# douban/tfmesos

Measured on AMD Instinct MI355X. Metric: global steps/sec, mnist_replica 1-ps/N-worker at 1/2/4/8 MI355X, higher is better.
Workload: dtype bf16; 1 GPU; model=mnist_replica_mlp_784x100x10, global_batch=100, parallelism=ps1+w1(colocated), optimizer=sgd, sync=True, transport=none(colocated-1proc)

## Files before the change

### tfmesos_amd/ops/csrc/gemm.hip

```cpp
#include <cstdlib>

#include "common.h"
#include "gemm.h"
#include "mlp_head.h"

namespace {

constexpr int BM = 64, BN = 64, BK = 32;
constexpr int SWZ_ELEMS = BM * BK;

DEVINL __bf16* sptr(__bf16* S, int r, int c) {
  return S + r * BK + ((((c >> 3) ^ ((r >> 2) & 3)) << 3) | (c & 7));
}
DEVINL const __bf16* sptr(const __bf16* S, int r, int c) {
  return S + r * BK + ((((c >> 3) ^ ((r >> 2) & 3)) << 3) | (c & 7));
}

typedef __attribute__((ext_vector_type(2))) __bf16 bf16x2;

DEVINL void stage_xk(const __bf16* __restrict__ P, __bf16* S,
                     int x0, int k0, int X, int K, int ld, int t, int vec) {
  const int x = t >> 2;
  const int kk0 = (t & 3) * 8;
  const int gx = x0 + x;
// ... 558 lines not shown
    for (int z2 = 0; z2 < nslice; ++z2)
      v += __builtin_bit_cast(
          float, *(const bf16x2*)&f1_smem[z2 * (G::WAVE_BYTES / 2) + e * 2]);
    if (bias != nullptr)
      v += e == t ? bv
                  : (bias_bf16 ? (float)((const __bf16*)bias)[col]
                               : ((const float*)bias)[col]);
    if (relu) v = v > 0.f ? v : 0.f;
    const long idx = (long)row * ldc + col;
    if (out_f32) ((float*)Cout)[idx] = v;
    else ((__bf16*)Cout)[idx] = (__bf16)v;
  }
}

typedef __attribute__((ext_vector_type(16))) float f32x16;

struct SmallSgd {
  float* pmw;
  bf16_t* psw;
  float* pmb;
  bf16_t* psb;
  const bf16_t* g2w;
  float* pm2w;
  bf16_t* ps2w;
  const bf16_t* g2b;
  float* pm2b;
  bf16_t* ps2b;
  float lr;
  int n2w, n2b;
};

DEVINL bf16x8 trs_frag(const __bf16* S, int ko, int lane) {
  const int kq = ko + ((lane & 15) >> 2);
  const int c = 16 * ((lane >> 4) & 1) + 4 * (lane & 3);
  bf16x4 f0 = tr_read(sptr(S, kq, c));
  bf16x4 f1 = tr_read(sptr(S, kq + 4, c));
  return __builtin_shufflevector(f0, f1, 0, 1, 2, 3, 4, 5, 6, 7);
}

DEVINL void small_cs_reduce(const float* csp, float* csw, int lane) {
  float c2[16];
#pragma unroll
  for (int j = 0; j < 16; ++j) c2[j] = csp[j];
#pragma unroll
  for (int off = 1; off < 32; off <<= 1)
#pragma unroll
    for (int j = 0; j < 16; ++j) c2[j] += __shfl_xor(c2[j], off, 64);
  if ((lane & 31) == 0) {
#pragma unroll
    for (int j = 0; j < 16; ++j) csw[(lane >> 5) * 16 + j] = c2[j];
  }
}

struct SmallSgdPre {
  float w[4];
  float b;
};

DEVINL void wait_vm0() { __builtin_amdgcn_s_waitcnt(0x0F70); }
DEVINL void wait_lgkm0() { __builtin_amdgcn_s_waitcnt(0xC07F); }

DEVINL int small_sgd_row(int m0, int w, int u, int lane) {
  const int v = w * 4 + u;
  return m0 + ((v >> 2) << 3) + ((lane >> 5) << 2) + (v & 3);
}

DEVINL void small_sgd_fetch(const SmallSgd& sg, SmallSgdPre& pre, bool cs,
                            int m0, int n0, int M, int N, int ldc, int w,
                            int lane) {
  const int n = n0 + (lane & 31);
#pragma unroll
  for (int u = 0; u < 4; ++u) {
    const int m = small_sgd_row(m0, w, u, lane);
    const long idx = (n < N && m < M) ? (long)m * ldc + n : 0;
    pre.w[u] = sg.pmw[idx];
  }
  pre.b = 0.f;
  if (cs && blockIdx.x == 0 && sg.pmb != nullptr) {
    const int nn = n0 + (lane & 31);
    pre.b = sg.pmb[nn < N ? nn : 0];
  }
}

DEVINL void small_sgd_fetch_buf(const SmallSgd& sg, SmallSgdPre& pre, int m0,
                                int n0, int M, int N, int w, int lane) {
  const brsrc_t wr = buf_rsrc(sg.pmw, M * N * 4);
  const int n = n0 + (lane & 31);
  const int nb = n < N ? n * 4 : BUF_OOB;
#pragma unroll
  for (int u = 0; u < 4; ++u)
    pre.w[u] = buf_f32(wr, nb + small_sgd_row(m0, w, u, lane) * N * 4);
  pre.b = 0.f;
  if (blockIdx.x == 0 && sg.pmb != nullptr)
    pre.b = buf_f32(buf_rsrc(sg.pmb, N * 4), n * 4);
}

DEVINL void small_sgd_commit(const SmallSgd& sg, const SmallSgdPre& pre,
                             const float (*red)[64 * 16],
                             const float (*csred)[32], bool cs, int m0,
                             int n0, int M, int N, int ldc, int w, int lane) {
  const int n = n0 + (lane & 31);
  if (n < N) {
#pragma unroll
    for (int u = 0; u < 4; ++u) {
      const int v = w * 4 + u;
      const int m = small_sgd_row(m0, w, u, lane);
      if (m >= M) continue;
      const float x = red[0][lane * 16 + v] + red[1][lane * 16 + v] +
                      red[2][lane * 16 + v] + red[3][lane * 16 + v];
      const long idx = (long)m * ldc + n;
      const float pv = pre.w[u] - sg.lr * x;
      sg.pmw[idx] = pv;
      sg.psw[idx] = f2bf(pv);
    }
  }
  if (cs && w == 0 && blockIdx.x == 0 && lane < 32) {
    const int nn = n0 + lane;
    if (nn < N && sg.pmb != nullptr) {
      const float sv = csred[0][lane] + csred[1][lane] + csred[2][lane] +
                       csred[3][lane];
      const float pv = pre.b - sg.lr * sv;
      sg.pmb[nn] = pv;
      sg.psb[nn] = f2bf(pv);
    }
  }
}

DEVINL void small_store(const float (*red)[64 * 16],
                        const float (*csred)[32], bool cs,
                        const void* bias, bool bias_bf16, void* Cout,
                        bool out_f32, int relu, void* colsum_out,
                        bool cs_f32, int m0, int n0, int M, int N, int ldc,
                        int lane) {
  f32x16 tot;
#pragma unroll
  for (int v = 0; v < 16; ++v)
    tot[v] = red[0][lane * 16 + v] + red[1][lane * 16 + v] +
             red[2][lane * 16 + v] + red[3][lane * 16 + v];
  const int n = n0 + (lane & 31);
  if (n < N) {
    float bvv = 0.f;
    if (bias != nullptr)
      bvv = bias_bf16 ? (float)((const __bf16*)bias)[n]
                      : ((const float*)bias)[n];
#pragma unroll
    for (int v = 0; v < 16; ++v) {
      const int m = m0 + ((v >> 2) << 3) + ((lane >> 5) << 2) + (v & 3);
      if (m >= M) continue;
      float x = tot[v] + bvv;
      if (relu) x = x > 0.f ? x : 0.f;
      if (out_f32) ((float*)Cout)[(long)m * ldc + n] = x;
      else ((__bf16*)Cout)[(long)m * ldc + n] = (__bf16)x;
    }
  }
  if (cs && blockIdx.x == 0 && lane < 32) {
    const int nn = n0 + lane;
    if (nn < N) {
      const float sv = csred[0][lane] + csred[1][lane] + csred[2][lane] +
                       csred[3][lane];
      if (cs_f32) ((float*)colsum_out)[nn] = sv;
      else ((__bf16*)colsum_out)[nn] = (__bf16)sv;
    }
  }
}

template <bool TA, bool CS>
__global__ __launch_bounds__(256)
void gemm_small_kernel(const __bf16* __restrict__ A,
                       const __bf16* __restrict__ B,
                       const void* __restrict__ bias, bool bias_bf16,
                       void* __restrict__ Cout, bool out_f32, int relu,
                       void* __restrict__ colsum_out, bool cs_f32,
                       int M, int N, int K, int lda, int ldb, int ldc,
                       int veca, int vecb, SmallSgd sg) {
  __shared__ __align__(16) __bf16 As[4][32 * BK];
  __shared__ __align__(16) __bf16 Bs[4][32 * BK];
  __shared__ float red[4][64 * 16];
  __shared__ float csred[4][32];
  const int t = threadIdx.x;
  const int lane = t & 63;
  const int w = t >> 6;
  const int m0 = blockIdx.x * 32;
  const int n0 = blockIdx.y * 32;
  const int kq = (((K + 3) / 4) + BK - 1) / BK * BK;
  const int ks = w * kq;
  const int ke = min(ks + kq, K);
  __bf16* Aw = As[w];
  __bf16* Bw = Bs[w];
  const int kk = lane & 31;
  const int half = lane >> 5;
  const bool av = veca == 8;
  const bool bv = vecb == 8;
  f32x4 acc[4] = {};
  float csp[16] = {};
  bf16x8 ra0, ra1, rb0, rb1;
  SmallSgdPre pre = {};
  if (sg.pmw != nullptr)
    small_sgd_fetch(sg, pre, CS, m0, n0, M, N, ldc, w, lane);

  auto load_a = [&](int k0) {
    ra0 = bf16x8{};
    ra1 = bf16x8{};
    if (TA) {
      const int gk = k0 + kk;
      const int gm = m0 + half * 16;
      if (gk < ke) {
        const __bf16* src = A + (long)gk * lda + gm;
        if (av && gm + 16 <= M && ((m0 & 7) == 0)) {
          ra0 = *(const bf16x8*)src;
          ra1 = *(const bf16x8*)(src + 8);
        } else {
#pragma unroll
          for (int j = 0; j < 8; ++j) {
            if (gm + j < M) ra0[j] = src[j];
            if (gm + 8 + j < M) ra1[j] = src[8 + j];
          }
        }
      }
    } else {
      const int gm = m0 + kk;
      const int gk0 = k0 + half * 16;
      if (gm < M) {
        const __bf16* src = A + (long)gm * lda + gk0;
        if (av && gk0 + 16 <= ke) {
          ra0 = *(const bf16x8*)src;
          ra1 = *(const bf16x8*)(src + 8);
        } else {
#pragma unroll
          for (int j = 0; j < 8; ++j) {
            if (gk0 + j < ke) ra0[j] = src[j];
            if (gk0 + 8 + j < ke) ra1[j] = src[8 + j];
          }
        }
      }
    }
    rb0 = bf16x8{};
    rb1 = bf16x8{};
    {
      const int gk = k0 + kk;
      const int gn = n0 + half * 16;
      if (gk < ke) {
        const __bf16* src = B + (long)gk * ldb + gn;
        if (bv && gn + 16 <= N && ((n0 & 7) == 0)) {
          rb0 = *(const bf16x8*)src;
          rb1 = *(const bf16x8*)(src + 8);
        } else {
// ... 48 lines not shown
    bf16x4 gv[4] = {};
    if (nv > 0) {
#pragma unroll
      for (int u = 0; u < 4; ++u) {
        const int i = lane + u * 64;
        gv[u] = ((const bf16x4*)sg.g2w)[i < nv ? i : 0];
        mv[u] = ((const f32x4*)sg.pm2w)[i < nv ? i : 0];
      }
    }
    const int it = (nv << 2) + lane;
    const int itc = it < sg.n2w ? it : 0;
    const int ibc = lane < sg.n2b ? lane : 0;
    const float mt = sg.pm2w[itc];
    const bf16_t gt = sg.g2w[itc];
    const float mb = sg.pm2b[ibc];
    const bf16_t gb = sg.g2b[ibc];
    wait_vm0();
#pragma unroll
    for (int u = 0; u < 4; ++u) {
      const int i = lane + u * 64;
      if (i < nv) {
        f32x4 pv;
        bf16x4 sv;
#pragma unroll
        for (int j = 0; j < 4; ++j) {
          pv[j] = mv[u][j] - sg.lr * (float)gv[u][j];
          sv[j] = (__bf16)pv[j];
        }
        ((f32x4*)sg.pm2w)[i] = pv;
        ((bf16x4*)sg.ps2w)[i] = sv;
      }
    }
    for (int i = 256 + lane; i < nv; i += 64) {
      f32x4 pv;
      bf16x4 sv;
      const bf16x4 g = ((const bf16x4*)sg.g2w)[i];
      const f32x4 m = ((const f32x4*)sg.pm2w)[i];
#pragma unroll
      for (int j = 0; j < 4; ++j) {
        pv[j] = m[j] - sg.lr * (float)g[j];
        sv[j] = (__bf16)pv[j];
      }
      ((f32x4*)sg.pm2w)[i] = pv;
      ((bf16x4*)sg.ps2w)[i] = sv;
    }
    if (it < sg.n2w) {
      const float pv = mt - sg.lr * bf2f(gt);
      sg.pm2w[it] = pv;
      sg.ps2w[it] = f2bf(pv);
    }
    if (lane < sg.n2b) {
      const float pv = mb - sg.lr * bf2f(gb);
      sg.pm2b[lane] = pv;
      sg.ps2b[lane] = f2bf(pv);
    }
    for (int i = lane + 64; i < sg.n2b; i += 64) {
      const float pv = sg.pm2b[i] - sg.lr * bf2f(sg.g2b[i]);
      sg.pm2b[i] = pv;
      sg.ps2b[i] = f2bf(pv);
    }
  }
  if (sg.pmw != nullptr) {
    small_sgd_commit(sg, pre, red, csred, CS, m0, n0, M, N, ldc, w, lane);
    return;
  }
  if (w != 0) return;
  small_store(red, csred, CS, bias, bias_bf16, Cout, out_f32, relu,
              colsum_out, cs_f32, m0, n0, M, N, ldc, lane);
}

struct HeadTail {
  const __bf16* h;
  const __bf16* w2;
  const bf16_t* b2;
  const long* labels;
  float* loss;
  void* dw2;
  void* db2;
  unsigned* ticket;
  float scale;
  int C;
};

template <bool APPLY, bool GF32, bool SNAP>
__global__ __launch_bounds__(256)
void mlp_head_tail_kernel(const __bf16* __restrict__ X, HeadTail ht,
                          void* __restrict__ Cout,
                          void* __restrict__ colsum_out,
                          int M, int N, int K, SmallSgd sg) {
  __shared__ __align__(16) __bf16 hs[HB * HP];
  __shared__ __align__(16) __bf16 wtp[4][CP * HP];
  __shared__ __align__(16) __bf16 wpd[4][32 * CP];
  __shared__ __align__(16) __bf16 dls[HB * CP];
  __shared__ float ls[HB * LSP];
  __shared__ float lsum[HB];
  __shared__ __align__(16) __bf16 As[4][32 * BK];
  __shared__ __align__(16) __bf16 Bs[4][32 * BK];
  __shared__ float red[4][64 * 16];
  __shared__ float csred[4][32];
  __shared__ float db2p[CP * 16];
  __shared__ unsigned tick;
  const int t = threadIdx.x;
  const int lane = t & 63;
  const int w = t >> 6;
  const int m0 = blockIdx.x * 32;
  const int n0 = blockIdx.y * 32;
  const int C = ht.C;
  const int ks = w * 32;
  const int ke = min(ks + 32, K);
  __bf16* Aw = As[w];
  __bf16* Bw = Bs[w];
  __bf16* wtw = wtp[w];
  __bf16* wpw = wpd[w];
  const int kk = lane & 31;
  const int half = lane >> 5;

  const int gk = ks + kk;
  const int gm = m0 + half * 16;
  const bool xvec = (M & 7) == 0;
  bf16x8 ra0 = {}, ra1 = {};
  unsigned xs[16];
  {
    const brsrc_t xr = buf_rsrc(X, K * M * 2);
    const int xrow = gk * M + gm;
    if (xvec) {
      ra0 = __builtin_bit_cast(bf16x8, __builtin_amdgcn_raw_buffer_load_b128(
          xr, gm < M ? xrow * 2 : BUF_OOB, 0, 0));
      ra1 = __builtin_bit_cast(bf16x8, __builtin_amdgcn_raw_buffer_load_b128(
          xr, gm + 8 < M ? (xrow + 8) * 2 : BUF_OOB, 0, 0));
    } else {
#pragma unroll
      for (int j = 0; j < 16; ++j)
        xs[j] = __builtin_amdgcn_raw_buffer_load_b16(
            xr, gm + j < M ? (xrow + j) * 2 : BUF_OOB, 0, 0);
    }
  }
  const int hc4 = kk * 4;
  bf16x4 hv[16];
  {
    const brsrc_t hr = buf_rsrc(ht.h, K * N * 2);
    const int hb = (hc4 < N ? hc4 * 2 : BUF_OOB) + (ks + half) * N * 2;
#pragma unroll
    for (int i = 0; i < 16; ++i)
      hv[i] = __builtin_bit_cast(bf16x4, __builtin_amdgcn_raw_buffer_load_b64(
          hr, hb + 2 * i * N * 2, 0, 0));
  }
  __bf16 wv[2][CP];
  bf16x8 wkm[4], wrow;
  if (SNAP) {
#pragma unroll
    for (int j = 0; j < 4; ++j) {
      const int q = lane + j * 64;
      wkm[j] = *(const bf16x8*)&ht.w2[kSnapKmajOff + (q >> 4) * HP +
                                      (q & 15) * 8];
    }
    wrow = *(const bf16x8*)&ht.w2[kSnapRowOff + n0 * CP + lane * 8];
  } else {
#pragma unroll
    for (int q = 0; q < 2; ++q) {
      const int hr = lane + q * 64;
#pragma unroll
      for (int c = 0; c < CP; ++c)
        wv[q][c] = ht.w2[(hr < N && c < C) ? hr * C + c : 0];
    }
  }
  const unsigned braw =
      __builtin_amdgcn_raw_buffer_load_b16(buf_rsrc(ht.b2, C * 2), kk * 2, 0, 0);
  const int label = (int)__builtin_amdgcn_raw_buffer_load_b32(
      buf_rsrc(ht.labels, K * 8), (ks + kk) * 8, 0, 0);
  SmallSgdPre pre = {};
  float pm2[16] = {};
  float pm2bv = 0.f;
  const bool snap_head =
      APPLY && SNAP && blockIdx.x == gridDim.x - 1 && blockIdx.y == 0;
  if (APPLY) {
    small_sgd_fetch_buf(sg, pre, m0, n0, M, N, w, lane);
    if (snap_head) {
      const brsrc_t w2r = buf_rsrc(sg.pm2w, N * C * 4);
      const int cb = kk < C ? kk * 4 : BUF_OOB;
#pragma unroll
      for (int v = 0; v < 16; ++v)
        pm2[v] = buf_f32(w2r, cb + (ks + head_frag_row(v, lane)) * C * 4);
      pm2bv = buf_f32(buf_rsrc(sg.pm2b, C * 4), t * 4);
    }
  }

  if (!SNAP) {
#pragma unroll
    for (int q = 0; q < 2; ++q)
#pragma unroll
      for (int c = 0; c < CP; ++c)
        if (!(lane + q * 64 < N && c < C)) wv[q][c] = (__bf16)0.f;
  }
  const float bc = __builtin_bit_cast(float, braw << 16);
  if (!xvec) {
    u32x4 d0, d1;
#pragma unroll
    for (int j = 0; j < 4; ++j) {
      d0[j] = xs[2 * j] | (xs[2 * j + 1] << 16);
      d1[j] = xs[8 + 2 * j] | (xs[9 + 2 * j] << 16);
    }
    ra0 = __builtin_bit_cast(bf16x8, d0);
    ra1 = __builtin_bit_cast(bf16x8, d1);
  }

  if (!SNAP) {
    const bf16x8 z8 = {};
    for (int i = lane * 8; i < CP * HP; i += 64 * 8) *(bf16x8*)&wtw[i] = z8;
    *(bf16x8*)&wpw[lane * 8] = z8;
  }
#pragma unroll
  for (int i = 0; i < 16; ++i)
    *(bf16x4*)&hs[(ks + 2 * i + half) * HP + hc4] = hv[i];
  if (SNAP) {
#pragma unroll
    for (int j = 0; j < 4; ++j) {
      const int q = lane + j * 64;
      *(bf16x8*)&wtw[(q >> 4) * HP + (q & 15) * 8] = wkm[j];
    }
    *(bf16x8*)&wpw[lane * 8] = wrow;
  } else {
#pragma unroll
    for (int q = 0; q < 2; ++q) {
      const int hr = lane + q * 64;
#pragma unroll
      for (int c = 0; c < CP; ++c) wtw[c * HP + hr] = wv[q][c];
      if (hr >= n0 && hr < n0 + 32 && hr < N) {
        bf16x8 lo, hi;
#pragma unroll
        for (int c = 0; c < 8; ++c) {
          lo[c] = wv[q][c];
          hi[c] = wv[q][8 + c];
        }
        *(bf16x8*)&wpw[(hr - n0) * CP] = lo;
        *(bf16x8*)&wpw[(hr - n0) * CP + 8] = hi;
      }
    }
  }

  {
    const f32x16v acc = head_logits_tile(
        &hs[(ks + kk) * HP], kk < CP ? &wtw[kk * HP] : nullptr, lane);
    head_store_logits(ls, acc, ks, bc, lane);
  }
  if (lane < 32) {
    const int row = ks + lane;
    const bf16x8 z8 = {};
    *(bf16x8*)&dls[row * CP] = z8;
    *(bf16x8*)&dls[row * CP + 8] = z8;
    float neglogp = 0.f;
    if (row < K)
      neglogp = head_softmax_row(
          &ls[row * LSP], C, label, ht.scale,
          [&](int c, float d) { dls[row * CP + c] = (__bf16)d; });
    lsum[row] = neglogp;
  }
  {
    const int colh = n0 + kk;
    __bf16 hm[16];
#pragma unroll
    for (int v = 0; v < 16; ++v)
      hm[v] = hs[(ks + head_frag_row(v, lane)) * HP + colh];
    const f32x16v acc =
        head_dh_tile(&dls[(ks + kk) * CP], &wpw[kk * CP], lane);
    wait_lgkm0();
#pragma unroll
    for (int v = 0; v < 16; ++v) {
      const int rl = head_frag_row(v, lane);
      const float hval = (float)hm[v];
      const float m =
          (ks + rl < K && colh < N && hval > 0.f) ? acc[v] : 0.f;
      const bf16_t r = f2bf(m);
      *sptr(Bw, rl, kk) = *(const __bf16*)&r;
    }
  }
  *(bf16x8*)sptr(Aw, kk, half * 16) = ra0;
  *(bf16x8*)sptr(Aw, kk, half * 16 + 8) = ra1;
  if (blockIdx.x == 0) {
    const bf16x8 rb0 = *(const bf16x8*)sptr(Bw, kk, half * 16);
    const bf16x8 rb1 = *(const bf16x8*)sptr(Bw, kk, half * 16 + 8);
    float csp[16] = {};
#pragma unroll
    for (int j = 0; j < 8; ++j) {
      csp[j] += (float)rb0[j];
      csp[8 + j] += (float)rb1[j];
    }
    small_cs_reduce(csp, csred[w], lane);
  }
  f32x4 acc[4] = {};
  if (ks < ke) {
#pragma unroll
    for (int kh = 0; kh < 2; ++kh) {
      const int ko = kh * 16 + ((lane >> 5) << 3);
      bf16x8 a = trs_frag(Aw, ko, lane);
      bf16x8 b = trs_frag(Bw, ko, lane);
      *(f32x16*)acc = __builtin_amdgcn_mfma_f32_32x32x16_bf16(
          a, b, *(f32x16*)acc, 0, 0, 0);
    }
  }
#pragma unroll
  for (int v = 0; v < 16; ++v) red[w][lane * 16 + v] = ((float*)acc)[v];
  __syncthreads();
  wait_vm0();

  bool head_block;
  constexpr bool ticketed = APPLY && !SNAP;
  if (APPLY) {
    if (ticketed && t == 0)
      tick = __hip_atomic_fetch_add(ht.ticket, 1u, __ATOMIC_ACQ_REL,
                                    __HIP_MEMORY_SCOPE_AGENT);
    small_sgd_commit(sg, pre, red, csred, true, m0, n0, M, N, N, w, lane);
    if (ticketed) {
      __syncthreads();
      head_block = tick == gridDim.x * gridDim.y - 1;
      if (head_block) {
#pragma unroll
        for (int v = 0; v < 16; ++v) {
          const int hrow = ks + head_frag_row(v, lane);
          pm2[v] = sg.pm2w[(kk < C && hrow < N) ? hrow * C + kk : 0];
        }
        pm2bv = sg.pm2b[t < C ? t : 0];
        wait_vm0();
      }
    } else {
      head_block = snap_head;
    }
  } else {
    if (gridDim.x * gridDim.y >= 32) {
      if (w == 0)
        small_store(red, csred, true, nullptr, false, Cout, GF32, 0,
                    colsum_out, GF32, m0, n0, M, N, N, lane);
    } else {
      const int wr = w >> 1, wc = w & 1;
      const int kfrag = (lane >> 4) * 8;
      const int kr = kfrag + ((lane & 15) >> 2);
      const int cq = 4 * (lane & 3);
      f32x4 c4 = {};
      for (int q = 0; q * 32 < K; ++q) {
        bf16x4 a0 = tr_read(sptr(As[q], kr, wr * 16 + cq));
        bf16x4 a1 = tr_read(sptr(As[q], kr + 4, wr * 16 + cq));
        bf16x4 b0 = tr_read(sptr(Bs[q], kr, wc * 16 + cq));
        bf16x4 b1 = tr_read(sptr(Bs[q], kr + 4, wc * 16 + cq));
        c4 = __builtin_amdgcn_mfma_f32_16x16x32_bf16(
            __builtin_shufflevector(a0, a1, 0, 1, 2, 3, 4, 5, 6, 7),
            __builtin_shufflevector(b0, b1, 0, 1, 2, 3, 4, 5, 6, 7), c4,
            0, 0, 0);
      }
      const int col = n0 + wc * 16 + (lane & 15);
      if (col < N) {
#pragma unroll
        for (int r = 0; r < 4; ++r) {
          const int row = m0 + wr * 16 + (lane >> 4) * 4 + r;
          if (row >= M) continue;
          float v = c4[r];
          v += 0.f;
          if (GF32) ((float*)Cout)[(long)row * N + col] = v;
          else ((__bf16*)Cout)[(long)row * N + col] = (__bf16)v;
        }
      }
      if (blockIdx.x == 0 && t < 32 && n0 + t < N) {
        float cs = 0.f;
        for (int q = 0; q * 32 < K; ++q)
#pragma unroll
          for (int k2 = 0; k2 < 32; ++k2) cs += (float)*sptr(Bs[q], k2, t);
        if (GF32) ((float*)colsum_out)[n0 + t] = cs;
        else ((__bf16*)colsum_out)[n0 + t] = (__bf16)cs;
      }
    }
    head_block = blockIdx.x == 0 && blockIdx.y == 0;
  }
  if (!head_block) return;

  {
    f32x16v acc2 = {};
    const int kr = (lane & 15) >> 2;
    const int ca = ks + 16 * ((lane >> 4) & 1) + 4 * (lane & 3);
    const int cb = 4 * (lane & 3);
    const bool bzero = ((lane >> 4) & 1) != 0;
#pragma unroll
    for (int kh = 0; kh < HB / 16; ++kh) {
      const int kq = kh * 16 + ((lane >> 5) << 3) + kr;
      bf16x4 a0 = tr_read(&hs[kq * HP + ca]);
      bf16x4 a1 = tr_read(&hs[(kq + 4) * HP + ca]);
      bf16x4 b0 = tr_read(&dls[kq * CP + cb]);
      bf16x4 b1 = tr_read(&dls[(kq + 4) * CP + cb]);
      bf16x8 a = __builtin_shufflevector(a0, a1, 0, 1, 2, 3, 4, 5, 6, 7);
      bf16x8 bv = __builtin_shufflevector(b0, b1, 0, 1, 2, 3, 4, 5, 6, 7);
      if (bzero) bv = bf16x8{};
      acc2 = __builtin_amdgcn_mfma_f32_32x32x16_bf16(a, bv, acc2, 0, 0, 0);
    }
    if (kk < C) {
#pragma unroll
      for (int v = 0; v < 16; ++v) {
        const int hrow = ks + head_frag_row(v, lane);
        if (hrow < N) {
          const int idx = hrow * C + kk;
          if (APPLY) {
            const float pv = pm2[v] - sg.lr * bf2f(f2bf(acc2[v]));
            sg.pm2w[idx] = pv;
            sg.ps2w[idx] = f2bf(pv);
          } else if (GF32) {
            ((float*)ht.dw2)[idx] = acc2[v];
          } else {
            ((bf16_t*)ht.dw2)[idx] = f2bf(acc2[v]);
          }
        }
      }
    }
  }
  if (t < C * 16) {
    const int c = t >> 4, part = t & 15;
    float s = 0.f;
    for (int b2 = part; b2 < K; b2 += 16) s += (float)dls[b2 * CP + c];
    db2p[t] = s;
  }
  __syncthreads();
  if (t < C) {
    float s = 0.f;
#pragma unroll
    for (int p2 = 0; p2 < 16; ++p2) s += db2p[t * 16 + p2];
    if (APPLY) {
      const float pv = pm2bv - sg.lr * bf2f(f2bf(s));
      sg.pm2b[t] = pv;
      sg.ps2b[t] = f2bf(pv);
    } else if (GF32) {
      ((float*)ht.db2)[t] = s;
    } else {
      ((bf16_t*)ht.db2)[t] = f2bf(s);
    }
  }
  if (w == 0) {
    float v = (lsum[lane] + 0.f) + (lsum[lane + 64] + 0.f);
#pragma unroll
    for (int s = 32; s > 0; s >>= 1) v += __shfl_down(v, s, 64);
    if (lane == 0) *ht.loss = v / K;
  }
  if (ticketed && t == 0)
    __hip_atomic_store(ht.ticket, 0u, __ATOMIC_RELAXED,
                       __HIP_MEMORY_SCOPE_AGENT);
}

__global__ __launch_bounds__(256)
void splitk_reduce_sgd_kernel(const float* __restrict__ ws, int nslice,
                              float* __restrict__ p,
                              __bf16* __restrict__ shadow, long mn,
                              float lr, float gscale, float nd) {
  const long i0 = ((long)blockIdx.x * blockDim.x + threadIdx.x) * 4;
  if (i0 >= mn) return;
  const bool vec4 = stripes_vec4(ws, mn);
  f32x4 v = {};
  for (int z = 0; z < nslice; ++z) {
    const float* sp = ws + (long)z * mn + i0;
    if (vec4) {
      const f32x4 sv = *(const f32x4*)sp;
#pragma unroll
      for (int j = 0; j < 4; ++j) v[j] += sv[j];
    } else {
#pragma unroll
      for (int j = 0; j < 4; ++j)
        if (i0 + j < mn) v[j] += sp[j];
    }
  }
#pragma unroll
  for (int j = 0; j < 4; ++j) {
    const long i = i0 + j;
    if (i >= mn) break;
    float pv = p[i];
    float g = gscale * v[j];
    if (nd != 0.f) g += nd * fminf(pv, 0.f);
    pv -= lr * g;
    p[i] = pv;
    if (shadow != nullptr) shadow[i] = (__bf16)pv;
  }
}

}

bool gemm_last_arriver(int M, int N, bool colsum, int act) {
  static int la_on = -1;
  if (la_on < 0) {
    const char* e = getenv("TFA_GEMM_LA");
    la_on = e ? atoi(e) : 0;
  }
  return la_on && !colsum && act <= 1 &&
         (long)ceil_div(N, BN) * ceil_div(M, BM) <= 64;
}

bool gemm_reduce_small(long mn) { return mn <= (1 << 16); }

void launch_gemm(const bf16_t* A, const bf16_t* B, const void* bias,
                 bool bias_bf16, void* C, bool out_f32, const bf16_t* aux,
                 void* colsum_out, float* ws, int* cnt, int kc, int nslice,
                 int M, int N, int K, int lda, int ldb, int ldc, bool ta,
                 bool tb, int act, int veca, int vecb, hipStream_t stream,
                 const SnapArgs* snap, bool* snap_taken) {
  SnapJob sj = {};
  if (snap_taken) *snap_taken = false;
  const bool sk = nslice > 1;
  dim3 grid(ceil_div(N, BN), ceil_div(M, BM), sk ? nslice : 1);
  dim3 block(256);
  const bool has_bias = bias != nullptr;
  const bool cs = colsum_out != nullptr;
  const int rflags = (act == 1 ? 1 : 0) | (out_f32 ? 2 : 0) |
                     (has_bias ? 4 : 0);
  if (!gemm_last_arriver(M, N, cs, act)) cnt = nullptr;
#define LAUNCH(TAv, TBv, ACTv, BIASv, OUTv, SKv, CSv)                       \
  hipLaunchKernelGGL((gemm_kernel<TAv, TBv, ACTv, BIASv, OUTv, SKv, CSv>),  \
                     grid, block, 0, stream, (const __bf16*)A,              \
                     (const __bf16*)B, bias, bias_bf16, C,                  \
                     (const __bf16*)aux, colsum_out, ws, cnt, M, N, K, lda, \
                     ldb, ldc, kc, veca, vecb, rflags)
  if (act == 2) {
    LAUNCH(false, true, 2, false, false, false, false);
    return;
  }
  if (act == 3) {
    LAUNCH(false, false, 3, false, false, false, false);
    return;
  }
  if (cs && !sk) {
    if (out_f32) LAUNCH(true, false, 0, false, true, false, true);
    else         LAUNCH(true, false, 0, false, false, false, true);
// ... 68 lines not shown
       else DISP_OUT(TAv, TBv, ACTv, false); } while (0)
#define DISP_ACT(TAv, TBv)                                                  \
  do { if (act == 1) DISP_BIAS(TAv, TBv, 1); else DISP_BIAS(TAv, TBv, 0); } while (0)
  if (ta) { if (tb) DISP_ACT(true, true); else DISP_ACT(true, false); }
  else    { if (tb) DISP_ACT(false, true); else DISP_ACT(false, false); }
#undef DISP_ACT
#undef DISP_BIAS
#undef DISP_OUT
#undef LAUNCH
}

void launch_gemm_fwd1(const bf16_t* A, const bf16_t* B, const void* bias,
                      bool bias_bf16, void* C, bool out_f32, int relu,
                      int kc, int nslice, int M, int N, int K, int lda,
                      int ldb, int ldc, int veca, int vecb, int variant,
                      const SnapArgs* snap, bool* snap_taken,
                      hipStream_t stream) {
  SnapJob sj = {};
  if (snap != nullptr) {
    sj.s0 = (const __bf16*)snap->s0; sj.s1 = (const __bf16*)snap->s1;
    sj.dst = (__bf16*)snap->dst;
    sj.n0 = snap->n0; sj.n1 = snap->n1; sj.off1 = snap->off1;
    sj.rows = snap->rows; sj.cols = snap->cols;
  }
  if (snap_taken) *snap_taken = snap != nullptr;
  if (variant < 0) variant = kFwd1Tile;
  const bool va = veca == 8 && K % 8 == 0;
  const bool vb = vecb >= 2 && N % 2 == 0 && N >= 8 && !(variant & 4);
  dim3 block(64 * nslice);
#define F1V(TMv, TNv, VAv, VBv)                                             \
  hipLaunchKernelGGL((gemm_fwd1_kernel<TMv, TNv, VAv, VBv>),                \
                     dim3(ceil_div(N, TNv), ceil_div(M, TMv)), block,       \
                     (nslice * (Fwd1Geo<TMv, TNv>::WAVE_BYTES)), stream,    \
                     (const __bf16*)A, (const __bf16*)B, bias, bias_bf16,   \
                     C, out_f32, relu, M, N, K, lda, ldb, ldc, kc, sj)
#define F1(TMv, TNv)                                                        \
  do { if (va) { if (vb) F1V(TMv, TNv, true, true);                         \
                 else F1V(TMv, TNv, true, false); }                         \
       else    { if (vb) F1V(TMv, TNv, false, true);                        \
                 else F1V(TMv, TNv, false, false); } } while (0)
  switch (variant & 3) {
    case 0: F1(16, 16); break;
    case 1: F1(16, 32); break;
    case 2: F1(32, 16); break;
    default: F1(32, 32); break;
  }
#undef F1
#undef F1V
}


void launch_gemm_small(const bf16_t* A, const bf16_t* B, const void* bias,
                       bool bias_bf16, void* C, bool out_f32, int relu,
                       void* colsum_out, bool cs_f32, int M, int N, int K,
                       int lda, int ldb, int ldc, bool ta, int veca,
                       int vecb, const SmallSgdArgs* sga,
                       hipStream_t stream) {
  dim3 grid(ceil_div(M, 32), ceil_div(N, 32)), block(256);
  SmallSgd sg = {};
  if (sga) {
    sg.pmw = sga->pmw; sg.psw = (bf16_t*)sga->psw;
    sg.pmb = sga->pmb; sg.psb = (bf16_t*)sga->psb;
    sg.g2w = (const bf16_t*)sga->g2w;
    sg.pm2w = sga->pm2w; sg.ps2w = (bf16_t*)sga->ps2w;
    sg.g2b = (const bf16_t*)sga->g2b;
    sg.pm2b = sga->pm2b; sg.ps2b = (bf16_t*)sga->ps2b;
    sg.lr = sga->lr; sg.n2w = sga->n2w; sg.n2b = sga->n2b;
  }
  const bool cs = colsum_out != nullptr || sg.pmb != nullptr;
#define GS(TAv, CSv)                                                        \
  hipLaunchKernelGGL((gemm_small_kernel<TAv, CSv>), grid, block, 0,         \
                     stream, (const __bf16*)A, (const __bf16*)B, bias,      \
                     bias_bf16, C, out_f32, relu, colsum_out, cs_f32, M, N, \
                     K, lda, ldb, ldc, veca, vecb, sg)
  if (ta) { if (cs) GS(true, true); else GS(true, false); }
  else    { if (cs) GS(false, true); else GS(false, false); }
#undef GS
}

void launch_mlp_head_tail(const bf16_t* x, const HeadTailArgs* hta,
                          void* dw1, void* db1, bool grads_f32, int M,
                          int H, int B, const SmallSgdArgs* sga,
                          hipStream_t stream) {
  dim3 grid(ceil_div(M, 32), ceil_div(H, 32)), block(256);
  HeadTail ht;
  ht.h = (const __bf16*)hta->h;
  ht.w2 = (const __bf16*)hta->w2;
  ht.b2 = (const bf16_t*)hta->b2;
  ht.labels = hta->labels;
  ht.loss = hta->loss;
  ht.dw2 = hta->dw2;
  ht.db2 = hta->db2;
  ht.ticket = hta->ticket;
  ht.scale = hta->scale;
  ht.C = hta->C;
  SmallSgd sg = {};
  if (sga) {
    sg.pmw = sga->pmw; sg.psw = (bf16_t*)sga->psw;
    sg.pmb = sga->pmb; sg.psb = (bf16_t*)sga->psb;
    sg.pm2w = sga->pm2w; sg.ps2w = (bf16_t*)sga->ps2w;
    sg.pm2b = sga->pm2b; sg.ps2b = (bf16_t*)sga->ps2b;
    sg.lr = sga->lr; sg.n2w = sga->n2w; sg.n2b = sga->n2b;
    if (ht.ticket == nullptr)
      hipLaunchKernelGGL((mlp_head_tail_kernel<true, false, true>), grid,
                         block, 0, stream, (const __bf16*)x, ht, nullptr,
                         nullptr, M, H, B, sg);
    else
      hipLaunchKernelGGL((mlp_head_tail_kernel<true, false, false>), grid,
                         block, 0, stream, (const __bf16*)x, ht, nullptr,
                         nullptr, M, H, B, sg);
  } else if (grads_f32) {
    hipLaunchKernelGGL((mlp_head_tail_kernel<false, true, false>), grid,
                       block, 0, stream, (const __bf16*)x, ht, dw1, db1, M, H,
                       B, sg);
  } else {
    hipLaunchKernelGGL((mlp_head_tail_kernel<false, false, false>), grid,
                       block, 0, stream, (const __bf16*)x, ht, dw1, db1, M, H,
                       B, sg);
  }
}


void launch_gemm_stripes_any(const bf16_t* A, const bf16_t* B, float* ws,
                             int kc, int nslice, int M, int N, int K,
                             int lda, int ldb, int ldc, bool ta, bool tb,
                             int veca, int vecb, hipStream_t stream) {
  const long Mtiles = ((long)M + BM - 1) / BM;
  dim3 grid((unsigned)ceil_div(N, BN), (unsigned)Mtiles, nslice);
  dim3 block(256);
#define SLAUNCH(TAv, TBv)                                                   \
  hipLaunchKernelGGL((gemm_kernel<TAv, TBv, 0, false, false, true, false>), \
                     grid, block, 0, stream, (const __bf16*)A,              \
                     (const __bf16*)B, nullptr, false, nullptr, nullptr,    \
                     nullptr, ws, nullptr, M, N, K, lda, ldb, ldc, kc, veca,\
                     vecb, 0)
  if (ta) { if (tb) SLAUNCH(true, true); else SLAUNCH(true, false); }
  else    { if (tb) SLAUNCH(false, true); else SLAUNCH(false, false); }
#undef SLAUNCH
}

void launch_splitk_reduce_sgd(const float* ws, int nslice, float* p,
                              bf16_t* shadow, long mn, float lr,
                              float gscale, float nd, hipStream_t stream) {
  dim3 rgrid((unsigned)(((mn + 3) / 4 + 255) / 256)), rblock(256);
  hipLaunchKernelGGL(splitk_reduce_sgd_kernel, rgrid, rblock, 0, stream,
                     ws, nslice, p, (__bf16*)shadow, mn, lr, gscale, nd);
}

void launch_gemm_stripes(const bf16_t* A, const bf16_t* B, float* ws,
                         int kc, int nslice, int M, int N, int K, int lda,
                         int ldb, int ldc, int veca, int vecb,
                         hipStream_t stream) {
  dim3 grid(ceil_div(N, BN), ceil_div(M, BM), nslice);
  dim3 block(256);
  hipLaunchKernelGGL((gemm_kernel<false, false, 0, false, false, true,
                                  false>),
                     grid, block, 0, stream, (const __bf16*)A,
                     (const __bf16*)B, nullptr, false, nullptr, nullptr,
                     nullptr, ws, nullptr, M, N, K, lda, ldb, ldc, kc,
                     veca, vecb, 0);
}
```

### tfmesos_amd/ops/csrc/mlp_head.h

```cpp
#pragma once

#include "common.h"

typedef __attribute__((ext_vector_type(16))) float f32x16v;

constexpr int HB = 128;
constexpr int HP = 136;
constexpr int CP = 16;
constexpr int LSP = CP + 1;

DEVINL int head_frag_row(int v, int lane) {
  return ((v >> 2) << 3) + ((lane >> 5) << 2) + (v & 3);
}

DEVINL f32x16v head_logits_tile(const __bf16* arow, const __bf16* brow,
                                int lane) {
  f32x16v acc = {};
#pragma unroll
  for (int kh = 0; kh < HB / 16; ++kh) {
    const int k0 = kh * 16 + ((lane >> 5) << 3);
    bf16x8 a = *(const bf16x8*)&arow[k0];
    bf16x8 bv = {};
    if (brow != nullptr) bv = *(const bf16x8*)&brow[k0];
    acc = __builtin_amdgcn_mfma_f32_32x32x16_bf16(a, bv, acc, 0, 0, 0);
  }
  return acc;
}

DEVINL void head_store_logits(float* ls, const f32x16v& acc, int row0,
                              float bc, int lane) {
  const int col = lane & 31;
  if (col < CP) {
#pragma unroll
    for (int v = 0; v < 16; ++v)
      ls[(row0 + head_frag_row(v, lane)) * LSP + col] = acc[v] + bc;
  }
}

template <class F>
DEVINL float head_softmax_row(const float* lr, int C, int label,
                              float scale, F emit) {
  float l[CP];
#pragma unroll
  for (int c = 0; c < CP; ++c) l[c] = lr[c];
  float mx = -3.4e38f;
#pragma unroll
  for (int c = 0; c < CP; ++c)
    if (c < C) mx = fmaxf(mx, l[c]);
  float sum = 0.f;
  float e[CP];
#pragma unroll
  for (int c = 0; c < CP; ++c) {
    e[c] = 0.f;
    if (c < C) {
      e[c] = __expf(l[c] - mx);
      sum += e[c];
    }
  }
  const float inv = 1.f / sum;
  float pl = 1.f;
  bool hit = false;
#pragma unroll
  for (int c = 0; c < CP; ++c) {
    if (c < C) {
      const float p = e[c] * inv;
      const float d = (p - (c == label ? 1.f : 0.f)) * scale;
      emit(c, d);
      if (c == label) {
        pl = p;
        hit = true;
      }
    }
  }
  return hit ? -__logf(fmaxf(pl, 1e-30f)) : 0.f;
}

DEVINL f32x16v head_dh_tile(const __bf16* drow, const __bf16* wrow,
                            int lane) {
  bf16x8 a = *(const bf16x8*)&drow[(lane >> 5) << 3];
  bf16x8 bv = *(const bf16x8*)&wrow[(lane >> 5) << 3];
  f32x16v acc = {};
  return __builtin_amdgcn_mfma_f32_32x32x16_bf16(a, bv, acc, 0, 0, 0);
}
```

Measured before the change: 56670 steps/s.

## Split fused MLP head-tail kernel into tile, db1 and classifier block roles

Restructures the fused backward head/tail kernel. For the non-ticketed (snapshot) path, it adds two extra grid columns whose blocks take dedicated roles: dW1 tiles, the db1 column-sum/SGD update, and the classifier dW2/db2 work split across two blocks. This keeps the serial head work off the last tile block. It also makes the softmax and logits paths branchless by padding classes with a negative-infinity bias and vectorized bf16 stores, and simplifies the dH masking writes. The cost is extra blocks that redundantly recompute the logits/softmax, plus more shared-memory padding.

New measurement: 65360 steps/s (median of 6 runs). +15.3%, better.

```diff
diff --git a/tfmesos_amd/ops/csrc/gemm.hip b/tfmesos_amd/ops/csrc/gemm.hip
--- a/tfmesos_amd/ops/csrc/gemm.hip
+++ b/tfmesos_amd/ops/csrc/gemm.hip
@@ -664,17 +664,34 @@
   }
 }
 
-DEVINL void small_sgd_fetch_buf(const SmallSgd& sg, SmallSgdPre& pre, int m0,
-                                int n0, int M, int N, int w, int lane) {
+DEVINL void small_sgd_fetch_buf_w(const SmallSgd& sg, SmallSgdPre& pre,
+                                  int m0, int n0, int M, int N, int w,
+                                  int lane) {
   const brsrc_t wr = buf_rsrc(sg.pmw, M * N * 4);
   const int n = n0 + (lane & 31);
   const int nb = n < N ? n * 4 : BUF_OOB;
 #pragma unroll
   for (int u = 0; u < 4; ++u)
     pre.w[u] = buf_f32(wr, nb + small_sgd_row(m0, w, u, lane) * N * 4);
-  pre.b = 0.f;
-  if (blockIdx.x == 0 && sg.pmb != nullptr)
-    pre.b = buf_f32(buf_rsrc(sg.pmb, N * 4), n * 4);
+}
+
+DEVINL void small_sgd_fetch_buf_b(const SmallSgd& sg, SmallSgdPre& pre,
+                                  int n0, int N, int lane) {
+  if (sg.pmb != nullptr)
+    pre.b = buf_f32(buf_rsrc(sg.pmb, N * 4), (n0 + (lane & 31)) * 4);
+}
+
+DEVINL void small_sgd_commit_b(const SmallSgd& sg, const SmallSgdPre& pre,
+                               const float (*csred)[32], int n0, int N,
+                               int lane) {
+  const int nn = n0 + lane;
+  if (nn < N && sg.pmb != nullptr) {
+    const float sv = csred[0][lane] + csred[1][lane] + csred[2][lane] +
+                     csred[3][lane];
+    const float pv = pre.b - sg.lr * sv;
+    sg.pmb[nn] = pv;
+    sg.psb[nn] = f2bf(pv);
+  }
 }
 
 DEVINL void small_sgd_commit(const SmallSgd& sg, const SmallSgdPre& pre,
@@ -696,15 +713,18 @@
       sg.psw[idx] = f2bf(pv);
     }
   }
-  if (cs && w == 0 && blockIdx.x == 0 && lane < 32) {
-    const int nn = n0 + lane;
-    if (nn < N && sg.pmb != nullptr) {
-      const float sv = csred[0][lane] + csred[1][lane] + csred[2][lane] +
-                       csred[3][lane];
-      const float pv = pre.b - sg.lr * sv;
-      sg.pmb[nn] = pv;
-      sg.psb[nn] = f2bf(pv);
-    }
+  if (cs && w == 0 && blockIdx.x == 0 && lane < 32)
+    small_sgd_commit_b(sg, pre, csred, n0, N, lane);
+}
+
+DEVINL void small_store_cs(const float (*csred)[32], void* colsum_out,
+                           bool cs_f32, int n0, int N, int lane) {
+  const int nn = n0 + lane;
+  if (nn < N) {
+    const float sv = csred[0][lane] + csred[1][lane] + csred[2][lane] +
+                     csred[3][lane];
+    if (cs_f32) ((float*)colsum_out)[nn] = sv;
+    else ((__bf16*)colsum_out)[nn] = (__bf16)sv;
   }
 }
 
@@ -735,15 +755,8 @@
       else ((__bf16*)Cout)[(long)m * ldc + n] = (__bf16)x;
     }
   }
-  if (cs && blockIdx.x == 0 && lane < 32) {
-    const int nn = n0 + lane;
-    if (nn < N) {
-      const float sv = csred[0][lane] + csred[1][lane] + csred[2][lane] +
-                       csred[3][lane];
-      if (cs_f32) ((float*)colsum_out)[nn] = sv;
-      else ((__bf16*)colsum_out)[nn] = (__bf16)sv;
-    }
-  }
+  if (cs && blockIdx.x == 0 && lane < 32)
+    small_store_cs(csred, colsum_out, cs_f32, n0, N, lane);
 }
 
 template <bool TA, bool CS>
@@ -958,24 +971,44 @@
   int C;
 };
 
-template <bool APPLY, bool GF32, bool SNAP>
-__global__ __launch_bounds__(256)
-void mlp_head_tail_kernel(const __bf16* __restrict__ X, HeadTail ht,
-                          void* __restrict__ Cout,
-                          void* __restrict__ colsum_out,
-                          int M, int N, int K, SmallSgd sg) {
-  __shared__ __align__(16) __bf16 hs[HB * HP];
-  __shared__ __align__(16) __bf16 wtp[4][CP * HP];
-  __shared__ __align__(16) __bf16 wpd[4][32 * CP];
-  __shared__ __align__(16) __bf16 dls[HB * CP];
-  __shared__ float ls[HB * LSP];
-  __shared__ float lsum[HB];
-  __shared__ __align__(16) __bf16 As[4][32 * BK];
-  __shared__ __align__(16) __bf16 Bs[4][32 * BK];
-  __shared__ float red[4][64 * 16];
-  __shared__ float csred[4][32];
-  __shared__ float db2p[CP * 16];
-  __shared__ unsigned tick;
+enum { HT_ALL = 0, HT_TILE = 1, HT_DB1 = 2, HT_CLS = 3 };
+
+struct HeadTailSmem {
+  alignas(16) __bf16 hs[HB * HP];
+  alignas(16) __bf16 wtp[4][(CP + 1) * HP];
+  alignas(16) __bf16 wpd[4][32 * CP];
+  alignas(16) __bf16 dls[HB * CP];
+  float ls[HB * LSP];
+  float lsum[HB];
+  alignas(16) __bf16 As[4][32 * BK];
+  alignas(16) __bf16 Bs[4][32 * BK];
+  float red[4][64 * 16];
+  float csred[4][32];
+  float db2p[CP * 16];
+  unsigned tick;
+};
+
+template <bool APPLY, bool GF32, bool SNAP, int ROLE>
+DEVINL void head_tail_body(HeadTailSmem& sm, const __bf16* __restrict__ X,
+                           const HeadTail& ht, void* __restrict__ Cout,
+                           void* __restrict__ colsum_out, int M, int N,
+                           int K, const SmallSgd& sg, int tiles) {
+  static_assert(ROLE != HT_ALL || (APPLY && !SNAP), "HT_ALL: ticket only");
+  static_assert(ROLE == HT_ALL || !APPLY || SNAP, "roles need no ticket");
+  constexpr bool TILE = ROLE == HT_ALL || ROLE == HT_TILE;
+  constexpr bool DH = ROLE != HT_CLS;
+  auto& hs = sm.hs;
+  auto& wtp = sm.wtp;
+  auto& wpd = sm.wpd;
+  auto& dls = sm.dls;
+  auto& ls = sm.ls;
+  auto& lsum = sm.lsum;
+  auto& As = sm.As;
+  auto& Bs = sm.Bs;
+  auto& red = sm.red;
+  auto& csred = sm.csred;
+  auto& db2p = sm.db2p;
+  auto& tick = sm.tick;
   const int t = threadIdx.x;
   const int lane = t & 63;
   const int w = t >> 6;
@@ -996,7 +1029,7 @@
   const bool xvec = (M & 7) == 0;
   bf16x8 ra0 = {}, ra1 = {};
   unsigned xs[16];
-  {
+  if (TILE) {
     const brsrc_t xr = buf_rsrc(X, K * M * 2);
     const int xrow = gk * M + gm;
     if (xvec) {
@@ -1030,7 +1063,7 @@
       wkm[j] = *(const bf16x8*)&ht.w2[kSnapKmajOff + (q >> 4) * HP +
                                       (q & 15) * 8];
     }
-    wrow = *(const bf16x8*)&ht.w2[kSnapRowOff + n0 * CP + lane * 8];
+    if (DH) wrow = *(const bf16x8*)&ht.w2[kSnapRowOff + n0 * CP + lane * 8];
   } else {
 #pragma unroll
     for (int q = 0; q < 2; ++q) {
@@ -1047,11 +1080,11 @@
   SmallSgdPre pre = {};
   float pm2[16] = {};
   float pm2bv = 0.f;
-  const bool snap_head =
-      APPLY && SNAP && blockIdx.x == gridDim.x - 1 && blockIdx.y == 0;
   if (APPLY) {
-    small_sgd_fetch_buf(sg, pre, m0, n0, M, N, w, lane);
-    if (snap_head) {
+    if (TILE) small_sgd_fetch_buf_w(sg, pre, m0, n0, M, N, w, lane);
+    if (ROLE == HT_DB1 || (ROLE == HT_ALL && blockIdx.x == 0))
+      small_sgd_fetch_buf_b(sg, pre, n0, N, lane);
+    if (ROLE == HT_CLS) {
       const brsrc_t w2r = buf_rsrc(sg.pm2w, N * C * 4);
       const int cb = kk < C ? kk * 4 : BUF_OOB;
 #pragma unroll
@@ -1068,8 +1101,9 @@
       for (int c = 0; c < CP; ++c)
         if (!(lane + q * 64 < N && c < C)) wv[q][c] = (__bf16)0.f;
   }
-  const float bc = __builtin_bit_cast(float, braw << 16);
-  if (!xvec) {
+  const float bc =
+      kk < C ? __builtin_bit_cast(float, braw << 16) : head_pad_bias();
+  if (TILE && !xvec) {
     u32x4 d0, d1;
 #pragma unroll
     for (int j = 0; j < 4; ++j) {
@@ -1083,25 +1117,26 @@
   if (!SNAP) {
     const bf16x8 z8 = {};
     for (int i = lane * 8; i < CP * HP; i += 64 * 8) *(bf16x8*)&wtw[i] = z8;
-    *(bf16x8*)&wpw[lane * 8] = z8;
+    if (DH) *(bf16x8*)&wpw[lane * 8] = z8;
   }
 #pragma unroll
   for (int i = 0; i < 16; ++i)
     *(bf16x4*)&hs[(ks + 2 * i + half) * HP + hc4] = hv[i];
+  if (lane < HB / 8) *(bf16x8*)&wtw[CP * HP + lane * 8] = bf16x8{};
   if (SNAP) {
 #pragma unroll
     for (int j = 0; j < 4; ++j) {
       const int q = lane + j * 64;
       *(bf16x8*)&wtw[(q >> 4) * HP + (q & 15) * 8] = wkm[j];
     }
-    *(bf16x8*)&wpw[lane * 8] = wrow;
+    if (DH) *(bf16x8*)&wpw[lane * 8] = wrow;
   } else {
 #pragma unroll
     for (int q = 0; q < 2; ++q) {
       const int hr = lane + q * 64;
 #pragma unroll
       for (int c = 0; c < CP; ++c) wtw[c * HP + hr] = wv[q][c];
-      if (hr >= n0 && hr < n0 + 32 && hr < N) {
+      if (DH && hr >= n0 && hr < n0 + 32 && hr < N) {
         bf16x8 lo, hi;
 #pragma unroll
         for (int c = 0; c < 8; ++c) {
@@ -1115,23 +1150,24 @@
   }
 
   {
-    const f32x16v acc = head_logits_tile(
-        &hs[(ks + kk) * HP], kk < CP ? &wtw[kk * HP] : nullptr, lane);
+    const f32x16v acc = head_logits_tile_all(
+        &hs[(ks + kk) * HP], &wtw[min(kk, CP) * HP], lane);
     head_store_logits(ls, acc, ks, bc, lane);
   }
   if (lane < 32) {
     const int row = ks + lane;
-    const bf16x8 z8 = {};
-    *(bf16x8*)&dls[row * CP] = z8;
-    *(bf16x8*)&dls[row * CP + 8] = z8;
     float neglogp = 0.f;
-    if (row < K)
-      neglogp = head_softmax_row(
-          &ls[row * LSP], C, label, ht.scale,
-          [&](int c, float d) { dls[row * CP + c] = (__bf16)d; });
+    if (row < K) {
+      neglogp = head_softmax_row_all(&ls[row * LSP], &dls[row * CP], C, label,
+                                     ht.scale);
+    } else {
+      const bf16x8 z8 = {};
+      *(bf16x8*)&dls[row * CP] = z8;
+      *(bf16x8*)&dls[row * CP + 8] = z8;
+    }
     lsum[row] = neglogp;
   }
-  {
+  if (DH) {
     const int colh = n0 + kk;
     __bf16 hm[16];
 #pragma unroll
@@ -1140,19 +1176,22 @@
     const f32x16v acc =
         head_dh_tile(&dls[(ks + kk) * CP], &wpw[kk * CP], lane);
     wait_lgkm0();
+    const int sw = (kk >> 3) ^ half;
+    __bf16* const bq[2] = {Bw + half * 4 * BK + (sw << 3) + (kk & 7),
+                           Bw + half * 4 * BK + ((sw ^ 2) << 3) + (kk & 7)};
 #pragma unroll
     for (int v = 0; v < 16; ++v) {
-      const int rl = head_frag_row(v, lane);
-      const float hval = (float)hm[v];
-      const float m =
-          (ks + rl < K && colh < N && hval > 0.f) ? acc[v] : 0.f;
+      const float m = (float)hm[v] > 0.f ? acc[v] : 0.f;
       const bf16_t r = f2bf(m);
-      *sptr(Bw, rl, kk) = *(const __bf16*)&r;
-    }
-  }
-  *(bf16x8*)sptr(Aw, kk, half * 16) = ra0;
-  *(bf16x8*)sptr(Aw, kk, half * 16 + 8) = ra1;
-  if (blockIdx.x == 0) {
+      bq[(v >> 2) & 1][((v >> 2) * 8 + (v & 3)) * BK] = *(const __bf16*)&r;
+    }
+  }
+  if (TILE) {
+    *(bf16x8*)sptr(Aw, kk, half * 16) = ra0;
+    *(bf16x8*)sptr(Aw, kk, half * 16 + 8) = ra1;
+  }
+  if (ROLE == HT_DB1 ? (APPLY || tiles >= 32)
+                     : (ROLE == HT_ALL && blockIdx.x == 0)) {
     const bf16x8 rb0 = *(const bf16x8*)sptr(Bw, kk, half * 16);
     const bf16x8 rb1 = *(const bf16x8*)sptr(Bw, kk, half * 16 + 8);
     float csp[16] = {};
@@ -1163,49 +1202,46 @@
     }
     small_cs_reduce(csp, csred[w], lane);
   }
-  f32x4 acc[4] = {};
-  if (ks < ke) {
-#pragma unroll
-    for (int kh = 0; kh < 2; ++kh) {
-      const int ko = kh * 16 + ((lane >> 5) << 3);
-      bf16x8 a = trs_frag(Aw, ko, lane);
-      bf16x8 b = trs_frag(Bw, ko, lane);
-      *(f32x16*)acc = __builtin_amdgcn_mfma_f32_32x32x16_bf16(
-          a, b, *(f32x16*)acc, 0, 0, 0);
-    }
-  }
-#pragma unroll
-  for (int v = 0; v < 16; ++v) red[w][lane * 16 + v] = ((float*)acc)[v];
+  if (TILE) {
+    f32x4 acc[4] = {};
+    if (ks < ke) {
+#pragma unroll
+      for (int kh = 0; kh < 2; ++kh) {
+        const int ko = kh * 16 + ((lane >> 5) << 3);
+        bf16x8 a = trs_frag(Aw, ko, lane);
+        bf16x8 b = trs_frag(Bw, ko, lane);
+        *(f32x16*)acc = __builtin_amdgcn_mfma_f32_32x32x16_bf16(
+            a, b, *(f32x16*)acc, 0, 0, 0);
+      }
+    }
+#pragma unroll
+    for (int v = 0; v < 16; ++v) red[w][lane * 16 + v] = ((float*)acc)[v];
+  }
   __syncthreads();
   wait_vm0();
 
-  bool head_block;
-  constexpr bool ticketed = APPLY && !SNAP;
-  if (APPLY) {
-    if (ticketed && t == 0)
+  constexpr bool ticketed = ROLE == HT_ALL;
+  if (ROLE == HT_ALL) {
+    if (t == 0)
       tick = __hip_atomic_fetch_add(ht.ticket, 1u, __ATOMIC_ACQ_REL,
                                     __HIP_MEMORY_SCOPE_AGENT);
     small_sgd_commit(sg, pre, red, csred, true, m0, n0, M, N, N, w, lane);
-    if (ticketed) {
-      __syncthreads();
-      head_block = tick == gridDim.x * gridDim.y - 1;
-      if (head_block) {
-#pragma unroll
-        for (int v = 0; v < 16; ++v) {
-          const int hrow = ks + head_frag_row(v, lane);
-          pm2[v] = sg.pm2w[(kk < C && hrow < N) ? hrow * C + kk : 0];
-        }
-        pm2bv = sg.pm2b[t < C ? t : 0];
-        wait_vm0();
-      }
-    } else {
-      head_block = snap_head;
-    }
-  } else {
-    if (gridDim.x * gridDim.y >= 32) {
+    __syncthreads();
+    if (tick != gridDim.x * gridDim.y - 1) return;
+#pragma unroll
+    for (int v = 0; v < 16; ++v) {
+      const int hrow = ks + head_frag_row(v, lane);
+      pm2[v] = sg.pm2w[(kk < C && hrow < N) ? hrow * C + kk : 0];
+    }
+    pm2bv = sg.pm2b[t < C ? t : 0];
+    wait_vm0();
+  } else if (ROLE == HT_TILE) {
+    if (APPLY) {
+      small_sgd_commit(sg, pre, red, csred, false, m0, n0, M, N, N, w, lane);
+    } else if (tiles >= 32) {
       if (w == 0)
-        small_store(red, csred, true, nullptr, false, Cout, GF32, 0,
-                    colsum_out, GF32, m0, n0, M, N, N, lane);
+        small_store(red, csred, false, nullptr, false, Cout, GF32, 0,
+                    nullptr, GF32, m0, n0, M, N, N, lane);
     } else {
       const int wr = w >> 1, wc = w & 1;
       const int kfrag = (lane >> 4) * 8;
@@ -1234,20 +1270,27 @@
           else ((__bf16*)Cout)[(long)row * N + col] = (__bf16)v;
         }
       }
-      if (blockIdx.x == 0 && t < 32 && n0 + t < N) {
-        float cs = 0.f;
-        for (int q = 0; q * 32 < K; ++q)
-#pragma unroll
-          for (int k2 = 0; k2 < 32; ++k2) cs += (float)*sptr(Bs[q], k2, t);
-        if (GF32) ((float*)colsum_out)[n0 + t] = cs;
-        else ((__bf16*)colsum_out)[n0 + t] = (__bf16)cs;
-      }
-    }
-    head_block = blockIdx.x == 0 && blockIdx.y == 0;
-  }
-  if (!head_block) return;
-
-  {
+    }
+    return;
+  } else if (ROLE == HT_DB1) {
+    if (APPLY) {
+      if (t < 32) small_sgd_commit_b(sg, pre, csred, n0, N, t);
+    } else if (tiles >= 32) {
+      if (t < 32) small_store_cs(csred, colsum_out, GF32, n0, N, t);
+    } else if (t < 32 && n0 + t < N) {
+      float cs = 0.f;
+      for (int q = 0; q * 32 < K; ++q)
+#pragma unroll
+        for (int k2 = 0; k2 < 32; ++k2) cs += (float)*sptr(Bs[q], k2, t);
+      if (GF32) ((float*)colsum_out)[n0 + t] = cs;
+      else ((__bf16*)colsum_out)[n0 + t] = (__bf16)cs;
+    }
+    return;
+  }
+  const bool do_dw2 = ROLE == HT_ALL || gridDim.y < 2 || blockIdx.y == 0;
+  const bool do_db2 = ROLE == HT_ALL || gridDim.y < 2 || blockIdx.y == 1;
+
+  if (do_dw2) {
     f32x16v acc2 = {};
     const int kr = (lane & 15) >> 2;
     const int ca = ks + 16 * ((lane >> 4) & 1) + 4 * (lane & 3);
@@ -1284,6 +1327,7 @@
       }
     }
   }
+  if (!do_db2) return;
   if (t < C * 16) {
     const int c = t >> 4, part = t & 15;
     float s = 0.f;
@@ -1314,6 +1358,31 @@
   if (ticketed && t == 0)
     __hip_atomic_store(ht.ticket, 0u, __ATOMIC_RELAXED,
                        __HIP_MEMORY_SCOPE_AGENT);
+}
+
+template <bool APPLY, bool GF32, bool SNAP>
+__global__ __launch_bounds__(256)
+void mlp_head_tail_kernel(const __bf16* __restrict__ X, HeadTail ht,
+                          void* __restrict__ Cout,
+                          void* __restrict__ colsum_out,
+                          int M, int N, int K, SmallSgd sg) {
+  __shared__ HeadTailSmem sm;
+  if constexpr (APPLY && !SNAP) {
+    head_tail_body<APPLY, GF32, SNAP, HT_ALL>(
+        sm, X, ht, Cout, colsum_out, M, N, K, sg, gridDim.x * gridDim.y);
+  } else {
+    const int mt = gridDim.x - 2;
+    const int tiles = mt * gridDim.y;
+    if ((int)blockIdx.x < mt)
+      head_tail_body<APPLY, GF32, SNAP, HT_TILE>(
+          sm, X, ht, Cout, colsum_out, M, N, K, sg, tiles);
+    else if ((int)blockIdx.x == mt)
+      head_tail_body<APPLY, GF32, SNAP, HT_DB1>(
+          sm, X, ht, Cout, colsum_out, M, N, K, sg, tiles);
+    else if (blockIdx.y < 2)
+      head_tail_body<APPLY, GF32, SNAP, HT_CLS>(
+          sm, X, ht, Cout, colsum_out, M, N, K, sg, tiles);
+  }
 }
 
 __global__ __launch_bounds__(256)
@@ -1548,7 +1617,8 @@
                           void* dw1, void* db1, bool grads_f32, int M,
                           int H, int B, const SmallSgdArgs* sga,
                           hipStream_t stream) {
-  dim3 grid(ceil_div(M, 32), ceil_div(H, 32)), block(256);
+  const bool roles = !(sga && hta->ticket != nullptr);
+  dim3 grid(ceil_div(M, 32) + (roles ? 2 : 0), ceil_div(H, 32)), block(256);
   HeadTail ht;
   ht.h = (const __bf16*)hta->h;
   ht.w2 = (const __bf16*)hta->w2;
diff --git a/tfmesos_amd/ops/csrc/mlp_head.h b/tfmesos_amd/ops/csrc/mlp_head.h
--- a/tfmesos_amd/ops/csrc/mlp_head.h
+++ b/tfmesos_amd/ops/csrc/mlp_head.h
@@ -75,6 +75,58 @@
   return hit ? -__logf(fmaxf(pl, 1e-30f)) : 0.f;
 }
 
+
+DEVINL f32x16v head_logits_tile_all(const __bf16* arow, const __bf16* brow,
+                                    int lane) {
+  bf16x8 a[HB / 16], bv[HB / 16];
+#pragma unroll
+  for (int kh = 0; kh < HB / 16; ++kh) {
+    const int k0 = kh * 16 + ((lane >> 5) << 3);
+    a[kh] = *(const bf16x8*)&arow[k0];
+    bv[kh] = *(const bf16x8*)&brow[k0];
+  }
+  f32x16v acc = {};
+#pragma unroll
+  for (int kh = 0; kh < HB / 16; ++kh)
+    acc = __builtin_amdgcn_mfma_f32_32x32x16_bf16(a[kh], bv[kh], acc, 0, 0, 0);
+  return acc;
+}
+
+DEVINL float head_pad_bias() { return -__builtin_inff(); }
+
+DEVINL float head_softmax_row_all(const float* lr, __bf16* drow, int C,
+                                  int label, float scale) {
+  float l[CP];
+#pragma unroll
+  for (int c = 0; c < CP; ++c) l[c] = lr[c];
+  const bool hit = (unsigned)label < (unsigned)C;
+  const int lab = hit ? label : 0;
+  const float ll = lr[lab];
+  float mx = -3.4e38f;
+#pragma unroll
+  for (int c = 0; c < CP; ++c) mx = fmaxf(mx, l[c]);
+  float sum = 0.f;
+  float e[CP];
+#pragma unroll
+  for (int c = 0; c < CP; ++c) {
+    e[c] = __expf(l[c] - mx);
+    sum += e[c];
+  }
+  const float inv = 1.f / sum;
+  bf16x8 lo, hi;
+#pragma unroll
+  for (int c = 0; c < 8; ++c) {
+    lo[c] = (__bf16)((e[c] * inv) * scale);
+    hi[c] = (__bf16)((e[8 + c] * inv) * scale);
+  }
+  *(bf16x8*)&drow[0] = lo;
+  *(bf16x8*)&drow[8] = hi;
+  const float el = __expf(ll - mx);
+  if (hit) drow[lab] = (__bf16)(__builtin_fmaf(el, inv, -1.f) * scale);
+  const float pl = el * inv;
+  return hit ? -__logf(fmaxf(pl, 1e-30f)) : 0.f;
+}
+
 DEVINL f32x16v head_dh_tile(const __bf16* drow, const __bf16* wrow,
                             int lane) {
   bf16x8 a = *(const bf16x8*)&drow[(lane >> 5) << 3];
```
